# yuhogun0908/MISOnet

Hardware: AMD Instinct MI355X
Metric: utterances/sec MISO1->MVDR->MISO3, 6-mic 16kHz 4s (higher is better)
Workload: dtype f32w; 1 GPU; BASELINE configs[3]: synthetic 6-mic 16 kHz 4 s, full MISO1x6 -> align -> MVDRx2 -> MISO3x2; batch_per_gpu=16, global_batch=16, frames=1001, freq_bins=129, parallelism=utterance-shard x1

## Files before the change

### misonet_amd/csrc/kernels.hpp

```cpp
#pragma once
#include <hip/hip_runtime.h>
#include <stdint.h>
#include <stdlib.h>
#include "det_stats.hpp"

namespace mn {

constexpr int CK = 8;
constexpr int TT = 128;
constexpr int TW = 136;
constexpr int FT = 4;
constexpr float IN_EPS = 1e-5f;
constexpr float GLN_EPS = 1e-8f;

#ifdef MISONET_EXPERIMENTS
inline int exp_env(const char* name, int dflt) { const char* e = getenv(name); return e ? atoi(e) : dflt; }
#else
constexpr int exp_env(const char*, int dflt) { return dflt; }
#endif

inline int round_up(int x, int m) { return (x + m - 1) / m * m; }
inline int frames_pitch(int T) { return round_up(T, 32); }

struct ConvArgs {
// ... 41 lines not shown
    const unsigned id = blockIdx.x;
    const unsigned xcd = id & 7u, k = id >> 3;
    const unsigned per = (unsigned)(a.ntx * a.nty * a.ncg);
    const unsigned grp = k / per;
    unsigned tile = k - grp * per;
    r.n = (int)(grp * 8u + xcd);
    r.t_tile = (int)(tile % (unsigned)a.ntx);
    tile /= (unsigned)a.ntx;
    r.cg = (int)(tile % (unsigned)a.ncg);
    r.f_tile = (int)(tile / (unsigned)a.ncg);
    r.valid = r.n < a.nsamp;
  } else {
    r.t_tile = blockIdx.x; r.f_tile = blockIdx.y;
    r.n = blockIdx.z / a.ncg; r.cg = blockIdx.z - r.n * a.ncg;
    r.valid = true;
  }
  return r;
}
inline dim3 conv_grid(ConvArgs& a, int n_samples, int tt, int ft, int xcd) {
  a.ntx = (a.T + tt - 1) / tt; a.nty = (a.Fout + ft - 1) / ft; a.nsamp = n_samples; a.xcd = xcd;
  if (xcd) return dim3((unsigned)(8 * ((n_samples + 7) / 8) * a.ntx * a.nty * a.ncg), 1, 1);
  return dim3(a.ntx, a.nty, n_samples * a.ncg);
}
int conv_xcd_env();
int device_cus();
int conv_cop(int Cout);
int conv_rows(int sf, int tr2);
hipError_t launch_conv(const ConvArgs& a, int n_samples, hipStream_t s);
hipError_t launch_conv_w1d(const ConvArgs& a, int n_samples, hipStream_t s);
hipError_t conv_init();
hipError_t launch_conv_wino(const ConvArgs& a, int n_samples, hipStream_t s);
hipError_t conv_wino_init();
hipError_t launch_conv_few(const ConvArgs& a, int n_samples, hipStream_t s);
hipError_t conv_few_init();
hipError_t launch_conv_wino6(const ConvArgs& a, int n_samples, hipStream_t s);
hipError_t conv_wino6_init();
hipError_t launch_conv_bf16(const ConvArgs& a, int n_samples, hipStream_t s);
hipError_t conv_bf16_init();
hipError_t launch_conv_bf16_dma(const ConvArgs& a, int n_samples, hipStream_t s);
hipError_t launch_conv_wprep(const ConvArgs& a, const float* wf, int n_samples, hipStream_t s);
hipError_t conv_bf16_dma_init();
hipError_t launch_conv_bf16x6(const ConvArgs& a, int n_samples, hipStream_t s);
hipError_t launch_conv_wprep6(const ConvArgs& a, const float* wf6, int n_samples, hipStream_t s);
hipError_t conv_bf16x6_init();
long long conv_bf16x6_wps_bytes(int Cin, int Cout);
hipError_t launch_conv_x6_first(const ConvArgs& a, const void* wimg, int n_samples, hipStream_t s);

int tcn_part_slots(int T);
hipError_t launch_tcn_prepare(const float* raw, long long raw_bstride, int raw_c0, const dstat_t* raw_stats, int raw_sstride,
                              float* x, double2* x_part, int C, int T, int Tp, int n_samples, hipStream_t s,
                              int raw_oct3 = 0);
hipError_t launch_tcn_dw(const float* x, const double2* x_part, int x_np, const float* wdw , const float* prelu ,
                         float* d, double2* gln_part , int C, int T, int Tp, int dilation, int n_samples, hipStream_t s,
                         int norm_kind = 0, const float* nsc = nullptr, const float* nsh = nullptr, const float2* fstat = nullptr);
hipError_t launch_tcn_cln_stats(const float* x, float2* fstat, int C, int T, int Tp, int n_samples, hipStream_t s);
hipError_t launch_tcn_pw(const float* d, const double2* gln_part, const float* gamma, const float* beta,
                         const float* wpw , const float* residual ,
                         float* y, long long y_bstride, int y_c0, double2* y_part , int C, int T, int Tp,
                         int n_samples, hipStream_t s,
                         int y_oct3_cbuf = 0, int x6 = 0);

hipError_t launch_pack(const float2* src, int B, int Mseg, int T, int F, float* dst, long long dst_bstride, int Tp,
                       int c_re, int c_im, int nshift, hipStream_t s);
hipError_t launch_unpack(const float* src, long long src_bstride, int Tp, int S, int T, int F, float2* dst, int n_samples,
                         int* nan_flag, hipStream_t s);
hipError_t launch_export(const float* src, long long src_bstride, int c0, int C, int Fq, int T, int Tp,
                         const dstat_t* stats, int sstride, int ident_c, float* dst, int n_samples, hipStream_t s,
                         int oct = 0);
hipError_t launch_unpack_ex(const float* src, long long src_bstride, int Tp, int S, int T, int F, int c_re0, int c_im0, int mode,
                            int M, const int* sel, float2* dst, int n_out, int* nan_flag, hipStream_t s);
hipError_t launch_compose_sel(const int* shift_sel, const int* clean_sel, int B, int M, int S, int* out, hipStream_t s);
hipError_t launch_assemble3(const float* in1, long long in1_bstride, const float* out1, long long out1_bstride,
                            const int* sel, int B, int M, int S, int ref_ch, int F, int Tp, float* in3,
                            long long in3_bstride, hipStream_t s);

hipError_t launch_stft_pack(const float* wav, int B, int L, int Mw, int T, const float* twid, float* dst,
                            long long dst_bstride, int Tp, int F, int c_re, int c_im, int nshift, hipStream_t s);
hipError_t stft_init();
void stft_build_twiddles(float* tw);
int stft_twiddle_count();
hipError_t launch_istft(const void* spec, int N, int T, const float* itw, short* out_i16, float* out_f32, hipStream_t s);
hipError_t istft_init();
void istft_build_twiddles(float* tw);
int istft_twiddle_count();

struct CView {
  const float* re; const float* im;
  long long sb, sf, sm; int st;
};
enum { BF_MVDR = 0, BF_SOUDEN = 1, BF_GEV = 2 };
struct MvdrArgs {
  CView mix;
  const float* est;
  long long est_bstride;
  const int* sel;
  CView src;
  int S;
  int B, F, M, T, Tp;
  float epsi;
  int kind = BF_MVDR;
  int noise_mix = 0;
  int trace_norm = 0;
  int ban = 0;
  int bf_ref = 0;
  double condition = 0.0;
};
long long mvdr_ws_bytes(int B, int S, int F, int M);
// ... 132 lines not shown
```

### misonet_amd/csrc/net.hip

```cpp
#include "net.hpp"

#include <math.h>
#include <cmath>
#include <algorithm>
#include <stdarg.h>
#include <stdio.h>
#include <stdlib.h>
#include <string.h>

using namespace mn;

static thread_local char g_err[512] = "";
int mn::fail(int code, const char* fmt, ...) {
  va_list ap;
  va_start(ap, fmt);
  vsnprintf(g_err, sizeof(g_err), fmt, ap);
  va_end(ap);
  return code;
}

Prof mn::g_profs[MAX_DEV];
std::atomic<int> mn::g_prof_any{0};

static int find_tensor(const misonet_net* n, const std::string& name) {
// ... 153 lines not shown
    }
  n->taps.push_back({"enc0_conv", B_E0, 0, en[0], false});
  for (int b = 0; b < 7; ++b) {
    snprintf(nm, sizeof(nm), "enc%d", b);
    n->taps.push_back({nm, B_D0 + (6 - b), de[6 - b], en[b], true});
  }
  n->taps.push_back({"tcn_out", B_D0, 0, 128, false});
  for (int i = 0; i < 6; ++i) {
    snprintf(nm, sizeof(nm), "dec%d", i);
    n->taps.push_back({nm, B_D0 + i + 1, 0, de[i + 1], true});
  }
  n->taps.push_back({"dec6", B_OUT, 0, c.out_ch, false});
  static const int x6first_env = exp_env("MISONET_X6_FIRST", 1);
  for (std::vector<ConvL>* v : {&n->enc, &n->dec})
    for (ConvL& l : *v)
      for (int mode = 0; mode < CONV_NMODES; ++mode) {
        const ConvShape sh = {l.Cin, l.Cout, n->bufs[l.in_buf].F, n->bufs[l.out_buf].F, l.sf, l.padf, l.tr2, l.act, l.transposed,
                              l.ident_c, l.in_buf == B_IN, buf_oct(mode, l.in_buf), buf_oct(mode, l.out_buf)};
        l.kind[mode] = conv_mode_built(mode) ? conv_select(sh, mode) : ConvKind::DIRECT;
        if (l.kind[mode] == ConvKind::X6_FIRST && !x6first_env) l.kind[mode] = ConvKind::DIRECT;
      }
  return MISONET_OK;
}

static inline long long buf_floats(const misonet_net* n, int Tp, int b) {
  const long long e = (long long)n->bufs[b].C * n->bufs[b].F * Tp;
  return buf_oct(n, b) == 3 ? e + e / 2 : e;
}
long long mn::bstride(const misonet_net* n, const Layout& L, int b) {
  if (b == B_IN && L.in_ext_off >= 0) return L.in_ext_bstride;
  return b >= B_TXA ? buf_floats(n, L.Tp, b) : L.sample_stride;
}

static void buf_lifetime(int b, int& t0, int& t1) {
  if (b == B_IN) { t0 = 0; t1 = 16; }
  else if (b >= B_E0 && b <= B_E4) { t0 = t1 = 1 + (b - B_E0); }
  else if (b >= B_D0 && b <= B_D6) { const int i = b - B_D0; t0 = 7 - i; t1 = 9 + i; }
  else if (b >= B_X2 && b <= B_X6) { t0 = t1 = 9 + 2 + (b - B_X2); }
  else { t0 = 15; t1 = 16; }
}

Layout mn::make_layout(const misonet_net* n, int N, int T, bool ext_in) {
  Layout L;
  L.N = N; L.T = T; L.Tp = frames_pitch(T);
  long long so = 0;
  for (int b = 0; b < NBUF; ++b) {
    L.stats_off[b] = so;
    so += (long long)N * n->bufs[b].C * 2 * DS_NL;
  }
  const long long tslots = tcn_part_slots(T);
  so = (so + 1) & ~1LL;
  L.tcn_xs = so;  so += 15LL * N * 128 * tslots * 2;
  L.tcn_ps = so;  so += 14LL * N * 128 * tslots * 2;
  L.tcn_gln = so; so += 28LL * N * 32 * 2;
  L.stats_doubles = so;
  L.data_base = align_up(256 + so * 8, 256);
  {
    struct Rect { int b, t0, t1; long long off, size; };
    std::vector<Rect> placed;
    std::vector<int> order;
    for (int b = 0; b < B_TXA; ++b)
      if (!(ext_in && b == B_IN)) order.push_back(b);
    L.data_off[B_IN] = 0;
    std::sort(order.begin(), order.end(), [&](int x, int y) {
      const long long sx = buf_floats(n, L.Tp, x), sy = buf_floats(n, L.Tp, y);
      return sx != sy ? sx > sy : x < y;
    });
    long long top = 0;
    for (int b : order) {
      Rect r;
      r.b = b;
      r.size = align_up(buf_floats(n, L.Tp, b), 64);
      buf_lifetime(b, r.t0, r.t1);
      if (n->keep_taps) { r.t0 = 0; r.t1 = 16; }
      std::vector<long long> cand(1, 0);
      for (const Rect& q : placed)
        if (q.t0 <= r.t1 && r.t0 <= q.t1) cand.push_back(q.off + q.size);
      std::sort(cand.begin(), cand.end());
      for (long long o : cand) {
        bool ok = true;
        for (const Rect& q : placed)
          if (q.t0 <= r.t1 && r.t0 <= q.t1 && o < q.off + q.size && q.off < o + r.size) { ok = false; break; }
        if (ok) { r.off = o; break; }
      }
      placed.push_back(r);
      L.data_off[b] = r.off;
      top = std::max(top, r.off + r.size);
    }
    L.sample_stride = top;
  }
  long long d = (long long)N * L.sample_stride;
  for (int b = B_TXA; b < NBUF; ++b) {
    L.data_off[b] = d;
    d += align_up((long long)N * buf_floats(n, L.Tp, b), 64);
  }
  long long wmax = 0, cmax = 0;
  auto scan = [&](const std::vector<ConvL>& v) {
    for (const ConvL& c : v) {
      const long long g = (c.Cout + 31) / 32, k = (c.Cin + 15) / 16;
      wmax = std::max(wmax, g * k * (2LL * 9 * 2 * 32 * 16));
      wmax = std::max(wmax, conv_bf16x6_wps_bytes((c.Cin + 7) / 8 * 8, c.Cout));
      cmax = std::max(cmax, g * 32);
    }
  };
  scan(n->enc); scan(n->dec);
  L.wps_base = align_up(L.data_base + d * 4, 256);
  L.wps_nstride = wmax;
// ... 76 lines not shown
      if (e == hipSuccess) { ProfScope ps(s, PK_CONV); e = launch_conv_bf16_dma(a, nb, s); }
      break;
    case ConvKind::WINO6: { a.ww6 = c.img(n->w_dev, kind); ProfScope ps(s, PK_CONV); e = launch_conv_wino6(a, nb, s); } break;
#endif
    default: e = hipErrorInvalidValue; break;
  }
  if (e == hipErrorInvalidValue)
    return fail(MISONET_EINVAL, "conv kernel kind %d refuses the layer Cin=%d Cout=%d Fin=%d Fout=%d sf=%d padf=%d tr2=%d act=%d in_oct=%d out_oct=%d (mode %d)",
                (int)kind, a.Cin, a.Cout, a.Fin, a.Fout, a.sf, a.padf, a.tr2, a.act, a.in_oct, a.out_oct, n->precision);
  HIPCHK(e);
  return MISONET_OK;
}

static unsigned layout_stamp(const misonet_net* n, const Layout& L) {
  unsigned h = 2166136261u;
  auto mix = [&](unsigned long long v) { for (int i = 0; i < 8; ++i) { h ^= (unsigned)(v & 0xff); h *= 16777619u; v >>= 8; } };
  mix(n->keep_taps ? 1 : 0); mix((unsigned)n->precision); mix((unsigned)L.N); mix((unsigned)L.T); mix((unsigned long long)L.total_bytes);
  return h | 1u;
}

int mn::forward_planar(misonet_net* n, const Layout& L, void* ws, hipStream_t s) {
  HIPCHK(hipMemsetAsync(ws, 0, (size_t)(256 + L.tcn_xs * 8), s));
  HIPCHK(hipMemsetD32Async(reinterpret_cast<hipDeviceptr_t>(reinterpret_cast<char*>(ws) + 8), (int)layout_stamp(n, L), 1, s));
  static const int sub_env = exp_env("MISONET_SUBBATCH", 0);
  auto run_stack = [&](const std::vector<ConvL>& v) -> int {
    if (sub_env <= 0) {
      for (const ConvL& c : v) { int r = run_conv(n, L, ws, c, s); if (r) return r; }
      return MISONET_OK;
    }
    size_t i = 0;
    while (i < v.size()) {
      const int Fg = n->bufs[v[i].out_buf].F;
      size_t j = i;
      while (j < v.size() && n->bufs[v[j].out_buf].F == Fg) ++j;
      int sb = sub_env * (127 / (Fg > 0 ? Fg : 1));
      if (sb < 1) sb = 1;
      for (int n0 = 0; n0 < L.N; n0 += sb) {
        const int nb = (L.N - n0) < sb ? (L.N - n0) : sb;
        for (size_t k = i; k < j; ++k) { int r = run_conv(n, L, ws, v[k], s, n0, nb); if (r) return r; }
      }
      i = j;
    }
    return MISONET_OK;
  };
  { int r = run_stack(n->enc); if (r) return r; }
  {
    ProfScope ps_tcn(s, PK_TCN);
    const int N = L.N, T = L.T, Tp = L.Tp;
    double2* xs = reinterpret_cast<double2*>(stats_base(ws) + L.tcn_xs);
    double2* ps = reinterpret_cast<double2*>(stats_base(ws) + L.tcn_ps);
    double2* gl = reinterpret_cast<double2*>(stats_base(ws) + L.tcn_gln);
    const int tslots = tcn_part_slots(T);
    const long long per = (long long)N * 128 * tslots;
    const long long gper = (long long)N * 32;
    float* xa = buf_ptr(L, ws, B_TXA);
    float* xb = buf_ptr(L, ws, B_TXB);
    float* td = buf_ptr(L, ws, B_TD);
    float* tp = buf_ptr(L, ws, B_TP);
    const int skip_c0 = n->cfg.de_ch[0];
    HIPCHK(launch_tcn_prepare(buf_ptr(L, ws, B_D0), bstride(n, L, B_D0), skip_c0, stats_ptr(L, ws, B_D0),
                              n->bufs[B_D0].C, xa, xs, 128, T, Tp, N, s, buf_oct(n, B_D0) == 3));
    float* cur = xa;
    float* nxt = xb;
    static const int tcn_x6_env = exp_env("MISONET_TCN_X6", 1);
    const int tcn_x6 = (n->precision == 3 && tcn_x6_env) ? 1 : 0;
    for (int k = 0; k < 14; ++k) {
      const TcnBlock& tb = n->tcn[k];
      const float* W = n->w_dev;
      const int nk = n->cfg.tcn_norm;
      float2* fstat = reinterpret_cast<float2*>(reinterpret_cast<char*>(ws) + L.fstat_base);
      if (nk == 2) HIPCHK(launch_tcn_cln_stats(cur, fstat, 128, T, Tp, N, s));
      HIPCHK(launch_tcn_dw(cur, xs + k * per, k == 0 ? 1 : tslots, W + tb.h[0].o_dw, W + tb.h[0].o_prelu, td, gl + (2 * k) * gper,
                           128, T, Tp, tb.dilation, N, s, nk, W + tb.h[0].o_nsc, W + tb.h[0].o_nsh, fstat));
      HIPCHK(launch_tcn_pw(td, gl + (2 * k) * gper, W + tb.h[0].o_gamma, W + tb.h[0].o_beta, W + tb.h[0].o_pw,
                           nullptr, tp, 128LL * Tp, 0, ps + k * per, 128, T, Tp, N, s, 0, tcn_x6));
      if (nk == 2) HIPCHK(launch_tcn_cln_stats(tp, fstat, 128, T, Tp, N, s));
      HIPCHK(launch_tcn_dw(tp, ps + k * per, tslots, W + tb.h[1].o_dw, W + tb.h[1].o_prelu, td,
                           gl + (2 * k + 1) * gper, 128, T, Tp, tb.dilation, N, s, nk, W + tb.h[1].o_nsc, W + tb.h[1].o_nsh, fstat));
      const bool last = (k == 13);
      float* y = last ? buf_ptr(L, ws, B_D0) : nxt;
      HIPCHK(launch_tcn_pw(td, gl + (2 * k + 1) * gper, W + tb.h[1].o_gamma, W + tb.h[1].o_beta,
                           W + tb.h[1].o_pw, cur, y, last ? bstride(n, L, B_D0) : 128LL * Tp, 0,
                           xs + (k + 1) * per, 128, T, Tp, N, s, (last && buf_oct(n, B_D0) == 3) ? n->bufs[B_D0].C : 0, tcn_x6));
      float* t = cur; cur = nxt; nxt = t;
    }
  }
  { int r = run_stack(n->dec); if (r) return r; }
  return MISONET_OK;
}

extern "C" {

const char* misonet_strerror(int code) {
  switch (code) {
    case MISONET_OK: return "ok";
    case MISONET_EINVAL: return "invalid argument / unsupported geometry";
    case MISONET_ESTATE: return "invalid call order or missing tensor";
    case MISONET_EHIP: return "HIP runtime error";
    case MISONET_ENOMEM: return "workspace too small";
    case MISONET_ENAN: return "NaN in network output";
    default: return "unknown error";
  }
}
const char* misonet_last_error(void) { return g_err; }
int misonet_version(void) { return 560; }

int misonet_net_create(const misonet_cfg* cfg, misonet_net** out) {
  if (!cfg || !out) return fail(MISONET_EINVAL, "null argument");
  misonet_net* n = new misonet_net();
  n->cfg = *cfg;
  int r = build_plan(n);
  if (r) { delete n; return r; }
  *out = n;
  return MISONET_OK;
}

int misonet_net_destroy(misonet_net* n) {
  if (!n) return MISONET_OK;
  if (n->w_dev) (void)hipFree(n->w_dev);
  delete n;
  return MISONET_OK;
}

int misonet_net_num_tensors(const misonet_net* n) { return n ? (int)n->tensors.size() : 0; }
const char* misonet_net_tensor_name(const misonet_net* n, int i) {
  if (!n || i < 0 || i >= (int)n->tensors.size()) return nullptr;
  return n->tensors[i].name.c_str();
}
long long misonet_net_tensor_numel(const misonet_net* n, int i) {
  if (!n || i < 0 || i >= (int)n->tensors.size()) return -1;
  return n->tensors[i].numel;
}

int misonet_net_set_tensor(misonet_net* n, const char* key, const float* host, long long numel) {
// ... 343 lines not shown
```

### misonet_amd/csrc/net.hpp

```cpp
#pragma once
#include "conv_select.hpp"
#include "api_common.hpp"

#include <string>

namespace mn {

struct Tensor {
  std::string name;
  long long numel;
  std::vector<float> host;
  bool set = false;
};

enum { B_IN = 0, B_E0, B_E1, B_E2, B_E3, B_E4, B_D0, B_D1, B_D2, B_D3, B_D4, B_D5, B_D6, B_X2, B_X3, B_X4, B_X5, B_X6,
       B_OUT, B_TXA, B_TXB, B_TD, B_TP, NBUF };

struct BufSpec { int C = 0, F = 0; };

struct ConvL {
  int in_buf, in_c0, Cin, ident_c;
  int out_buf, out_c0, Cout;
  int sf, padf, tr2, act;
  bool transposed;
  int wt, bt;
  int cop, ncg;
  ConvKind kind[CONV_NMODES];
  long long img_off[CONV_NKIND];
  long long b_off = 0;
  float wscale = 1.f;
  const float* img(const float* w_dev, ConvKind k) const { return w_dev + img_off[(int)k]; }
};

struct TcnHalf {
  int dw, prelu, gamma, beta, pw; long long o_dw, o_prelu, o_gamma, o_beta, o_pw;
  int on[4] = {-1, -1, -1, -1};
  long long o_nsc = 0, o_nsh = 0;
};
struct TcnBlock { int dilation; TcnHalf h[2]; };

struct Tap { std::string name; int buf, c0, C; bool normalised; };

struct Layout {
  int N, T, Tp;
  long long data_off[NBUF];
  long long sample_stride;
  long long in_ext_off = -1;
  long long in_ext_bstride = 0;
  long long stats_off[NBUF];
  long long tcn_xs, tcn_ps, tcn_gln;
  long long stats_doubles;
  long long data_base;
  long long wps_base, wps_nstride;
  long long btab_base, btab_nstride;
  long long fstat_base;
  long long total_bytes;
};

}

struct misonet_net {
  misonet_cfg cfg;
  int S;
  mn::BufSpec bufs[mn::NBUF];
  std::vector<mn::Tensor> tensors;
  std::vector<mn::ConvL> enc, dec;
  std::vector<mn::TcnBlock> tcn;
  std::vector<mn::Tap> taps;
  float* w_dev = nullptr;
  bool committed = false;
  bool keep_taps = false;
  int precision = 3;
};

namespace mn {

inline long long align_up(long long x, long long a) { return (x + a - 1) / a * a; }

Layout make_layout(const misonet_net* n, int N, int T, bool ext_in = false);
long long bstride(const misonet_net* n, const Layout& L, int b);
inline float* buf_ptr(const Layout& L, void* ws, int b) {
  if (b == B_IN && L.in_ext_off >= 0) return reinterpret_cast<float*>(reinterpret_cast<char*>(ws) + L.in_ext_off);
  return reinterpret_cast<float*>(reinterpret_cast<char*>(ws) + L.data_base) + L.data_off[b];
}
int forward_planar(misonet_net* n, const Layout& L, void* ws, hipStream_t s);

}
```

### misonet_amd/csrc/tcn.hip

```cpp
#include "kernels.hpp"
#include "conv_epilogue.hpp"

namespace mn {

typedef float f32x16 __attribute__((ext_vector_type(16)));

__device__ inline double block_sum_256(double v, double* s_tmp ) {
#pragma unroll
  for (int m = 32; m >= 1; m >>= 1) v += __shfl_xor(v, m, 64);
  const int tid = threadIdx.x;
  __syncthreads();
  if ((tid & 63) == 0) s_tmp[tid >> 6] = v;
  __syncthreads();
  return s_tmp[0] + s_tmp[1] + s_tmp[2] + s_tmp[3];
}

__device__ inline double2 tpart_sum(const double2* p, int np) {
  double2 s = p[0];
#pragma unroll 8
  for (int i = 1; i < np; ++i) { const double2 q = p[i]; s.x += q.x; s.y += q.y; }
  return s;
}

__device__ inline void in_params(double2 st, int T, float& mean, float& rstd) {
  const double m = st.x / (double)T;
  double var = st.y / (double)T - m * m;
  var = var > 0.0 ? var : 0.0;
  mean = (float)m;
  rstd = (float)(1.0 / sqrt(var + (double)IN_EPS));
}

__global__ __launch_bounds__(256) void tcn_prepare_k(const float* raw, long long raw_bstride, int raw_c0,
                                                     const dstat_t* raw_stats, int raw_sstride, float* x,
                                                     double2* x_part, int nps, int C, int T, int Tp, int raw_oct3) {
  __shared__ double s_tmp[4];
  const int c = blockIdx.x, n = blockIdx.y;
  float mean, rstd;
  {
    const dstat_t* st = raw_stats + ((long long)n * raw_sstride + raw_c0 + c) * (2 * DS_NL);
    in_params(make_double2(dstat_read(st), dstat_read(st + DS_NL)), T, mean, rstd);
  }
  const float* src = raw + (long long)n * raw_bstride + (long long)(raw_c0 + c) * Tp;
  const unsigned short* so = reinterpret_cast<const unsigned short*>(raw + (long long)n * raw_bstride);
  const int ch = raw_c0 + c;
  const long long part_e = (long long)(raw_sstride >> 3) * Tp * 8;
  float* dst = x + ((long long)n * C + c) * Tp;
  double s1 = 0.0, s2 = 0.0;
  for (int t = threadIdx.x; t < T; t += 256) {
    float r;
    if (raw_oct3) {
      const long long e = ((long long)(ch >> 3) * Tp + t) * 8 + (ch & 7);
      r = (__uint_as_float((unsigned)so[e] << 16) + __uint_as_float((unsigned)so[part_e + e] << 16)) +
          __uint_as_float((unsigned)so[2 * part_e + e] << 16);
    } else {
      r = src[t];
    }
    const float v = (r - mean) * rstd;
    dst[t] = v;
    s1 += v;
    s2 += (double)v * v;
  }
  s1 = block_sum_256(s1, s_tmp);
  s2 = block_sum_256(s2, s_tmp);
  if (threadIdx.x == 0) x_part[((long long)n * C + c) * nps] = make_double2(s1, s2);
}

constexpr int DW_MAXT = 2048;
constexpr int DW_HALO = 64;
constexpr int DW_SEG = DW_MAXT - 2 * DW_HALO;
template <int NORM>
__global__ __launch_bounds__(256) void tcn_dw_k(const float* x, const double2* x_part, int x_np, int nps,
                                                const float* wdw, const float* prelu, float* d, double2* gln_part,
                                                int C, int T, int Tp, int dil, int seg_f, const float* nsc, const float* nsh,
                                                const float2* fstat) {
  __shared__ double s_tmp[4][2];
  extern __shared__ __align__(16) float s_a_dyn[];
  const int row_f = seg_f + 2 * DW_HALO;
  const int lane = threadIdx.x & 63, wave = threadIdx.x >> 6;
  const int c = blockIdx.x * 4 + wave, n = blockIdx.y;
  float sc, sh, mu = 0.f;
  if (NORM == 0) {
    float mean, rstd;
    in_params(tpart_sum(x_part + ((long long)n * C + c) * nps, x_np), T, mean, rstd);
    sc = rstd; sh = 0.f; mu = mean;
  } else if (NORM == 1) {
    __shared__ double s_g[4];
    double a1 = 0.0, a2 = 0.0;
    for (int r = threadIdx.x; r < C; r += 256) {
      const double2 q = tpart_sum(x_part + ((long long)n * C + r) * nps, x_np);
      a1 += q.x; a2 += q.y;
    }
    a1 = block_sum_256(a1, s_g);
    a2 = block_sum_256(a2, s_g);
    const double cnt = (double)C * (double)T;
    const double gm = a1 / cnt;
    double gv = a2 / cnt - gm * gm;
    gv = gv > 0.0 ? gv : 0.0;
    const float rstd = (float)(1.0 / sqrt(gv + (double)GLN_EPS));
    sc = nsc[c] * rstd;
    sh = nsh[c];
    mu = (float)gm;
  } else if (NORM == 3) {
    sc = nsc[c]; sh = nsh[c];
  } else {
    sc = nsc[c]; sh = nsh[c];
  }
  const float2* fs = NORM == 2 ? fstat + (long long)n * Tp : nullptr;
  const float w0 = wdw[c * 3 + 0], w1 = wdw[c * 3 + 1], w2 = wdw[c * 3 + 2];
  const float slope = prelu[0];
  const float* src = x + ((long long)n * C + c) * Tp;
  float* dst = d + ((long long)n * C + c) * Tp;
  float* a = s_a_dyn + wave * row_f;
  const int Tq = (T + 3) & ~3;
  double r1 = 0.0, r2 = 0.0;
  for (int ts = 0; ts < Tq; ts += seg_f) {
    if (ts) __syncthreads();
    for (int j = lane * 4; j < row_f; j += 256) {
      const int t = ts - DW_HALO + j;
      float4 o = make_float4(0.f, 0.f, 0.f, 0.f);
      if (t >= 0 && t < Tq) {
        float4 v = *reinterpret_cast<const float4*>(src + t);
        if (NORM == 2) {
          const float4 f01 = *reinterpret_cast<const float4*>(fs + t), f23 = *reinterpret_cast<const float4*>(fs + t + 2);
          v.x = (v.x - f01.x) * f01.y; v.y = (v.y - f01.z) * f01.w;
          v.z = (v.z - f23.x) * f23.y; v.w = (v.w - f23.z) * f23.w;
        }
        o.x = (t + 0 < T) ? elu_fast(fmaf(v.x - mu, sc, sh)) : 0.f;
        o.y = (t + 1 < T) ? elu_fast(fmaf(v.y - mu, sc, sh)) : 0.f;
        o.z = (t + 2 < T) ? elu_fast(fmaf(v.z - mu, sc, sh)) : 0.f;
        o.w = (t + 3 < T) ? elu_fast(fmaf(v.w - mu, sc, sh)) : 0.f;
      }
      *reinterpret_cast<float4*>(a + j) = o;
    }
    __syncthreads();
    const int te = (ts + seg_f < Tq) ? ts + seg_f : Tq;
    float s1 = 0.f, s2 = 0.f;
    for (int t = ts + lane * 4; t < te; t += 256) {
      float o[4];
#pragma unroll
      for (int i = 0; i < 4; ++i) {
        const int tc = t + i;
        const int j = tc - ts + DW_HALO;
        float acc = w1 * a[j];
        acc = fmaf(w0, a[j - dil], acc);
        acc = fmaf(w2, a[j + dil], acc);
        acc = acc > 0.f ? acc : slope * acc;
        o[i] = acc;
        if (tc < T) { s1 += acc; s2 = fmaf(acc, acc, s2); }
      }
      *reinterpret_cast<float4*>(dst + t) = make_float4(o[0], o[1], o[2], o[3]);
    }
    r1 += (double)s1;
    r2 += (double)s2;
  }
// ... 193 lines not shown
  __amdgpu_buffer_rsrc_t rs_o[3];
  {
    const unsigned long long po = reinterpret_cast<unsigned long long>(y) + (unsigned long long)n * y_bstride * 4ull +
                                  (unsigned long long)(y_c0 >> 3) * OP16;
    const unsigned long long pb = (unsigned long long)(y_cbuf >> 3) * OP16;
    const unsigned nrec = Y_OCT3 ? (unsigned)(C >> 3) * OP16 : 0u;
    rs_o[0] = make_rsrc_e(po, nrec);
    rs_o[1] = make_rsrc_e(po + pb, nrec);
    rs_o[2] = make_rsrc_e(po + 2 * pb, nrec);
  }
  float s1[16], s2[16], piv[16];
#pragma unroll
  for (int r = 0; r < 16; ++r) {
    s1[r] = 0.f; s2[r] = 0.f;
    piv[r] = __shfl(acc[0][r] + rv[0][r], lane & 32, 64);
  }
#pragma unroll
  for (int s = 0; s < 4; ++s) {
    const int t = t0 + s * 32 + l31;
    const bool ok = t < T;
    const float m = ok ? 1.f : 0.f;
    const unsigned vo = ok ? (unsigned)((wave * 32 + 4 * half) * Tp + t) * 4u : 0x80000000u;
    float vrow[16];
#pragma unroll
    for (int r = 0; r < 16; ++r) {
      const int co_off = (r & 3) + 8 * (r >> 2);
      const float v = acc[s][r] + rv[s][r];
      vrow[r] = v;
      if (!Y_OCT3)
        __builtin_amdgcn_raw_buffer_store_b32(__builtin_bit_cast(unsigned, v), rs_y, vo + (unsigned)(co_off * Tp) * 4u, 0, 0);
      const float vm = (v - piv[r]) * m;
      s1[r] += vm;
      s2[r] = fmaf(vm, vm, s2[r]);
    }
    if (Y_OCT3)
      store_oct_row<3>(vrow, rs_o, (unsigned)t * 16u + (unsigned)(4 * wave + half) * OP16, OP16, ok, ok);
  }
  if (y_part) {
    const float x1 = reduce16_halfwave(s1, lane);
    const float x2 = reduce16_halfwave(s2, lane);
    if ((lane & 16) == 0) {
      const int q = lane & 15;
      const int co = wave * 32 + (q & 3) + 8 * (q >> 2) + 4 * half;
      float pq = piv[0];
#pragma unroll
      for (int r = 1; r < 16; ++r) pq = (q == r) ? piv[r] : pq;
      const double c = (double)pq, S1 = (double)x1, S2 = (double)x2;
      const double nv = (double)((T - t0) < PW_TT ? (T - t0) : PW_TT);
      y_part[((long long)n * C + co) * nps + blockIdx.x] = make_double2(S1 + nv * c, S2 + 2.0 * c * S1 + nv * c * c);
    }
  }
}

int tcn_part_slots(int T) { return (T + PW_TT - 1) / PW_TT; }

hipError_t launch_tcn_prepare(const float* raw, long long raw_bstride, int raw_c0, const dstat_t* raw_stats,
                              int raw_sstride, float* x, double2* x_part, int C, int T, int Tp, int n_samples,
                              hipStream_t s, int raw_oct3) {
  hipLaunchKernelGGL(tcn_prepare_k, dim3(C, n_samples), dim3(256), 0, s, raw, raw_bstride, raw_c0, raw_stats,
                     raw_sstride, x, x_part, tcn_part_slots(T), C, T, Tp, raw_oct3);
  return hipGetLastError();
}

__global__ __launch_bounds__(256) void tcn_cln_stats_k(const float* x, float2* fstat, int C, int T, int Tp) {
  const int t = blockIdx.x * 256 + threadIdx.x, n = blockIdx.y;
  if (t >= Tp) return;
  float2 o = make_float2(0.f, 0.f);
  if (t < T) {
    const float* p = x + (long long)n * C * Tp + t;
    float m = 0.f;
    for (int c = 0; c < C; ++c) m += p[(long long)c * Tp];
    m /= (float)C;
    float v = 0.f;
    for (int c = 0; c < C; ++c) { const float dd = p[(long long)c * Tp] - m; v = fmaf(dd, dd, v); }
    v /= (float)C;
    o = make_float2(m, 1.f / sqrtf(v + GLN_EPS));
  }
  fstat[(long long)n * Tp + t] = o;
}

hipError_t launch_tcn_cln_stats(const float* x, float2* fstat, int C, int T, int Tp, int n_samples, hipStream_t s) {
  hipLaunchKernelGGL(tcn_cln_stats_k, dim3((Tp + 255) / 256, n_samples), dim3(256), 0, s, x, fstat, C, T, Tp);
  return hipGetLastError();
}

hipError_t launch_tcn_dw(const float* x, const double2* x_part, int x_np, const float* wdw, const float* prelu, float* d,
                         double2* gln_part, int C, int T, int Tp, int dilation, int n_samples, hipStream_t s, int norm_kind,
                         const float* nsc, const float* nsh, const float2* fstat) {
  if (dilation < 1 || dilation > DW_HALO) return hipErrorInvalidValue;
  if (C % 4) return hipErrorInvalidValue;
  if (norm_kind < 0 || norm_kind > 3 || (norm_kind && (!nsc || !nsh)) || (norm_kind == 2 && !fstat)) return hipErrorInvalidValue;
  const int tq = (T + 3) & ~3;
  const int seg_f = tq < DW_SEG ? tq : DW_SEG;
  const dim3 g(C / 4, n_samples);
  const size_t lds = (size_t)4 * (seg_f + 2 * DW_HALO) * sizeof(float);
#define MN_DW(K) hipLaunchKernelGGL(tcn_dw_k<K>, g, dim3(256), lds, s, x, x_part, x_np, tcn_part_slots(T), wdw, prelu, d, gln_part, \
                                    C, T, Tp, dilation, seg_f, nsc, nsh, fstat)
  if (norm_kind == 0) MN_DW(0); else if (norm_kind == 1) MN_DW(1); else if (norm_kind == 2) MN_DW(2); else MN_DW(3);
#undef MN_DW
  return hipGetLastError();
}

hipError_t launch_tcn_pw(const float* d, const double2* gln_part, const float* gamma, const float* beta,
                         const float* wpw, const float* residual, float* y, long long y_bstride, int y_c0,
                         double2* y_part, int C, int T, int Tp, int n_samples, hipStream_t s, int y_oct3_cbuf, int x6) {
  if (C != 128) return hipErrorInvalidValue;
  const dim3 g((T + PW_TT - 1) / PW_TT, n_samples);
  const int nps = tcn_part_slots(T);
  if (y_oct3_cbuf) {
    if ((y_c0 & 7) || (y_oct3_cbuf & 7)) return hipErrorInvalidValue;
    if (x6) hipLaunchKernelGGL((tcn_pw_k<true, true>), g, dim3(256), 0, s, d, gln_part, gamma, beta, wpw, residual, y,
                               y_bstride, y_c0, y_part, nps, T, Tp, y_oct3_cbuf);
    else hipLaunchKernelGGL((tcn_pw_k<true, false>), g, dim3(256), 0, s, d, gln_part, gamma, beta, wpw, residual, y,
                            y_bstride, y_c0, y_part, nps, T, Tp, y_oct3_cbuf);
  } else {
    if (x6) hipLaunchKernelGGL((tcn_pw_k<false, true>), g, dim3(256), 0, s, d, gln_part, gamma, beta, wpw, residual, y,
                               y_bstride, y_c0, y_part, nps, T, Tp, 0);
    else hipLaunchKernelGGL((tcn_pw_k<false, false>), g, dim3(256), 0, s, d, gln_part, gamma, beta, wpw, residual, y,
                            y_bstride, y_c0, y_part, nps, T, Tp, 0);
  }
  return hipGetLastError();
}

}
```

Before: 149.1 utt/s.

## Fuse first TCN depthwise conv with pointwise conv, defer gLN into next norm

Adds a fused kernel that computes the first half-block's depthwise conv, PReLU and gamma scaling in LDS and feeds it straight into the pointwise MFMA GEMM. This removes the intermediate depthwise activation round-trip through global memory and one launch per TCN block. The global-LayerNorm statistics are folded algebraically into the following depthwise kernel's instance-norm scale (new NORM==4 path), using pivot-shifted partial sums for numerical stability. Beta is dropped, which is valid only because the next instance norm cancels per-channel offsets. The cost is a larger, more register- and LDS-hungry kernel and a more fragile chain of statistics.

```diff
diff --git a/misonet_amd/csrc/kernels.hpp b/misonet_amd/csrc/kernels.hpp
--- a/misonet_amd/csrc/kernels.hpp
+++ b/misonet_amd/csrc/kernels.hpp
@@ -117,7 +117,12 @@
                               int raw_oct3 = 0);
 hipError_t launch_tcn_dw(const float* x, const double2* x_part, int x_np, const float* wdw , const float* prelu ,
                          float* d, double2* gln_part , int C, int T, int Tp, int dilation, int n_samples, hipStream_t s,
-                         int norm_kind = 0, const float* nsc = nullptr, const float* nsh = nullptr, const float2* fstat = nullptr);
+                         int norm_kind = 0, const float* nsc = nullptr, const float* nsh = nullptr, const float2* fstat = nullptr,
+                         const double2* p_gln = nullptr);
+hipError_t launch_tcn_ds(const float* x, const double2* x_part, int x_np, const float* wdw , const float* prelu ,
+                         const float* gamma, const float* wpw, float* p, double2* p_part ,
+                         double2* gln_part , int C, int T, int Tp, int dilation, int n_samples, hipStream_t s,
+                         int x6 = 0, const double2* pivot_gln = nullptr);
 hipError_t launch_tcn_cln_stats(const float* x, float2* fstat, int C, int T, int Tp, int n_samples, hipStream_t s);
 hipError_t launch_tcn_pw(const float* d, const double2* gln_part, const float* gamma, const float* beta,
                          const float* wpw , const float* residual ,
diff --git a/misonet_amd/csrc/net.hip b/misonet_amd/csrc/net.hip
--- a/misonet_amd/csrc/net.hip
+++ b/misonet_amd/csrc/net.hip
@@ -229,7 +229,8 @@
   so = (so + 1) & ~1LL;
   L.tcn_xs = so;  so += 15LL * N * 128 * tslots * 2;
   L.tcn_ps = so;  so += 14LL * N * 128 * tslots * 2;
-  L.tcn_gln = so; so += 28LL * N * 32 * 2;
+  L.tcn_g0 = (int)std::max(32LL, tslots);
+  L.tcn_gln = so; so += 14LL * N * (L.tcn_g0 + 32) * 2;
   L.stats_doubles = so;
   L.data_base = align_up(256 + so * 8, 256);
   {
@@ -412,7 +413,8 @@
     double2* gl = reinterpret_cast<double2*>(stats_base(ws) + L.tcn_gln);
     const int tslots = tcn_part_slots(T);
     const long long per = (long long)N * 128 * tslots;
-    const long long gper = (long long)N * 32;
+    const long long g0per = (long long)N * L.tcn_g0;
+    const long long gper = g0per + (long long)N * 32;
     float* xa = buf_ptr(L, ws, B_TXA);
     float* xb = buf_ptr(L, ws, B_TXB);
     float* td = buf_ptr(L, ws, B_TD);
@@ -424,22 +426,33 @@
     float* nxt = xb;
     static const int tcn_x6_env = exp_env("MISONET_TCN_X6", 1);
     const int tcn_x6 = (n->precision == 3 && tcn_x6_env) ? 1 : 0;
+    static const int tcn_fuse = exp_env("MISONET_TCN_FUSE", 1);
     for (int k = 0; k < 14; ++k) {
       const TcnBlock& tb = n->tcn[k];
       const float* W = n->w_dev;
       const int nk = n->cfg.tcn_norm;
       float2* fstat = reinterpret_cast<float2*>(reinterpret_cast<char*>(ws) + L.fstat_base);
       if (nk == 2) HIPCHK(launch_tcn_cln_stats(cur, fstat, 128, T, Tp, N, s));
-      HIPCHK(launch_tcn_dw(cur, xs + k * per, k == 0 ? 1 : tslots, W + tb.h[0].o_dw, W + tb.h[0].o_prelu, td, gl + (2 * k) * gper,
-                           128, T, Tp, tb.dilation, N, s, nk, W + tb.h[0].o_nsc, W + tb.h[0].o_nsh, fstat));
-      HIPCHK(launch_tcn_pw(td, gl + (2 * k) * gper, W + tb.h[0].o_gamma, W + tb.h[0].o_beta, W + tb.h[0].o_pw,
-                           nullptr, tp, 128LL * Tp, 0, ps + k * per, 128, T, Tp, N, s, 0, tcn_x6));
-      if (nk == 2) HIPCHK(launch_tcn_cln_stats(tp, fstat, 128, T, Tp, N, s));
-      HIPCHK(launch_tcn_dw(tp, ps + k * per, tslots, W + tb.h[1].o_dw, W + tb.h[1].o_prelu, td,
-                           gl + (2 * k + 1) * gper, 128, T, Tp, tb.dilation, N, s, nk, W + tb.h[1].o_nsc, W + tb.h[1].o_nsh, fstat));
+      double2* g0 = gl + k * gper;
+      double2* g1 = g0 + g0per;
+      if (nk == 0 && tcn_fuse) {
+        HIPCHK(launch_tcn_ds(cur, xs + k * per, k == 0 ? 1 : tslots, W + tb.h[0].o_dw, W + tb.h[0].o_prelu, W + tb.h[0].o_gamma,
+                             W + tb.h[0].o_pw, tp, ps + k * per, g0, 128, T, Tp, tb.dilation, N, s, tcn_x6,
+                             k ? g0 - gper : nullptr));
+        HIPCHK(launch_tcn_dw(tp, ps + k * per, tslots, W + tb.h[1].o_dw, W + tb.h[1].o_prelu, td, g1, 128, T, Tp, tb.dilation,
+                             N, s, 4, nullptr, nullptr, nullptr, g0));
+      } else {
+        HIPCHK(launch_tcn_dw(cur, xs + k * per, k == 0 ? 1 : tslots, W + tb.h[0].o_dw, W + tb.h[0].o_prelu, td, g0,
+                             128, T, Tp, tb.dilation, N, s, nk, W + tb.h[0].o_nsc, W + tb.h[0].o_nsh, fstat));
+        HIPCHK(launch_tcn_pw(td, g0, W + tb.h[0].o_gamma, W + tb.h[0].o_beta, W + tb.h[0].o_pw,
+                             nullptr, tp, 128LL * Tp, 0, ps + k * per, 128, T, Tp, N, s, 0, tcn_x6));
+        if (nk == 2) HIPCHK(launch_tcn_cln_stats(tp, fstat, 128, T, Tp, N, s));
+        HIPCHK(launch_tcn_dw(tp, ps + k * per, tslots, W + tb.h[1].o_dw, W + tb.h[1].o_prelu, td,
+                             g1, 128, T, Tp, tb.dilation, N, s, nk, W + tb.h[1].o_nsc, W + tb.h[1].o_nsh, fstat));
+      }
       const bool last = (k == 13);
       float* y = last ? buf_ptr(L, ws, B_D0) : nxt;
-      HIPCHK(launch_tcn_pw(td, gl + (2 * k + 1) * gper, W + tb.h[1].o_gamma, W + tb.h[1].o_beta,
+      HIPCHK(launch_tcn_pw(td, g1, W + tb.h[1].o_gamma, W + tb.h[1].o_beta,
                            W + tb.h[1].o_pw, cur, y, last ? bstride(n, L, B_D0) : 128LL * Tp, 0,
                            xs + (k + 1) * per, 128, T, Tp, N, s, (last && buf_oct(n, B_D0) == 3) ? n->bufs[B_D0].C : 0, tcn_x6));
       float* t = cur; cur = nxt; nxt = t;
diff --git a/misonet_amd/csrc/net.hpp b/misonet_amd/csrc/net.hpp
--- a/misonet_amd/csrc/net.hpp
+++ b/misonet_amd/csrc/net.hpp
@@ -49,6 +49,7 @@
   long long in_ext_bstride = 0;
   long long stats_off[NBUF];
   long long tcn_xs, tcn_ps, tcn_gln;
+  int tcn_g0;
   long long stats_doubles;
   long long data_base;
   long long wps_base, wps_nstride;
diff --git a/misonet_amd/csrc/tcn.hip b/misonet_amd/csrc/tcn.hip
--- a/misonet_amd/csrc/tcn.hip
+++ b/misonet_amd/csrc/tcn.hip
@@ -72,7 +72,7 @@
 __global__ __launch_bounds__(256) void tcn_dw_k(const float* x, const double2* x_part, int x_np, int nps,
                                                 const float* wdw, const float* prelu, float* d, double2* gln_part,
                                                 int C, int T, int Tp, int dil, int seg_f, const float* nsc, const float* nsh,
-                                                const float2* fstat) {
+                                                const float2* fstat, const double2* p_gln) {
   __shared__ double s_tmp[4][2];
   extern __shared__ __align__(16) float s_a_dyn[];
   const int row_f = seg_f + 2 * DW_HALO;
@@ -100,6 +100,20 @@
     sc = nsc[c] * rstd;
     sh = nsh[c];
     mu = (float)gm;
+  } else if (NORM == 4) {
+    const double2 st = tpart_sum(x_part + ((long long)n * C + c) * nps, x_np);
+    const double2 gs = tpart_sum(p_gln + (long long)n * nps, nps);
+    const double cnt = (double)C * (double)T;
+    const double gm = gs.x / cnt;
+    double gv = gs.y / cnt - gm * gm;
+    gv = gv < 0.0 ? 0.0 : gv;
+    const double r = 1.0 / sqrt(gv + (double)GLN_EPS);
+    const double m = st.x / (double)T;
+    double var = st.y / (double)T - m * m;
+    var = var < 0.0 ? 0.0 : var;
+    mu = (float)m;
+    sc = (float)(r / sqrt(r * r * var + (double)IN_EPS));
+    sh = 0.f;
   } else if (NORM == 3) {
     sc = nsc[c]; sh = nsh[c];
   } else {
@@ -399,7 +413,304 @@
   }
 }
 
+constexpr int DS_AW = PW_TT + 2 * DW_HALO;
+
+__device__ __forceinline__ float4 ds_row4(const float* p, bool al4) {
+  if (al4) return *reinterpret_cast<const float4*>(p);
+  return make_float4(p[0], p[1], p[2], p[3]);
+}
+
+__device__ __forceinline__ float ds_tap(float slope, float ac, float al, float ar, float4 cw) {
+  float acc = cw.y * ac;
+  acc = fmaf(cw.x, al, acc);
+  acc = fmaf(cw.z, ar, acc);
+  return acc > 0.f ? acc : slope * acc;
+}
+
+__device__ __forceinline__ float ds_keep(float v, unsigned mask) {
+  return __builtin_bit_cast(float, __builtin_bit_cast(unsigned, v) & mask);
+}
+
+template <bool X6>
+__global__ __launch_bounds__(256) void tcn_ds_k(const float* x, const double2* x_part, int x_np, int nps, const float* wdw,
+                                                const float* prelu, const float* gamma, const float* wt ,
+                                                float* y, double2* y_part, double2* gln_part, int T, int Tp, int dil,
+                                                const double2* piv_part) {
+  constexpr int C = 128;
+  __shared__ __align__(16) float s_a[PW_KC][DS_AW];
+  __shared__ __align__(16) float4 s_cw[C];
+  __shared__ float2 s_in[C];
+  __shared__ double s_red[4][2];
+  const int tid = threadIdx.x, lane = tid & 63, wave = tid >> 6;
+  const int half = lane >> 5, l31 = lane & 31;
+  const int t0 = blockIdx.x * PW_TT, n = blockIdx.y;
+  const float* xn = x + (long long)n * C * Tp;
+  if (tid < C) {
+    float mean, rstd;
+    in_params(tpart_sum(x_part + ((long long)n * C + tid) * nps, x_np), T, mean, rstd);
+    s_in[tid] = make_float2(mean, rstd);
+    s_cw[tid] = make_float4(wdw[tid * 3 + 0], wdw[tid * 3 + 1], wdw[tid * 3 + 2], gamma[tid]);
+  }
+  const float slope = prelu[0];
+  const bool al4 = (dil & 3) == 0;
+  const float cpv = piv_part ? (float)(tpart_sum(piv_part + (long long)n * nps, nps).x / ((double)C * (double)T)) : 0.f;
+  const int ec = tid >> 4, eq = tid & 15;
+  const int qlo = (DW_HALO - dil) >> 2, qhi = (DW_HALO + PW_TT + dil + 3) >> 2;
+  const int ni = (qhi - qlo + 15) >> 4;
+  const int tq0 = t0 - DW_HALO + 4 * (qlo + eq), tq1 = tq0 + 64, tq2 = tq0 + 128, tq3 = tq0 + 192;
+  const float* xe = xn + ec * Tp;
+  const float* xp0 = xe + ((unsigned)tq0 < (unsigned)Tp ? tq0 : 0);
+  const float* xp1 = xe + ((unsigned)tq1 < (unsigned)Tp ? tq1 : 0);
+  const float* xp2 = xe + ((unsigned)tq2 < (unsigned)Tp ? tq2 : 0);
+  const float* xp3 = xe + ((unsigned)tq3 < (unsigned)Tp ? tq3 : 0);
+  float* ae = &s_a[ec][4 * (qlo + eq)];
+  float4 xr0, xr1, xr2, xr3 = make_float4(0.f, 0.f, 0.f, 0.f);
+#define DS_XISSUE(K0)                                                                                            \
+  {                                                                                                              \
+    const int ko_ = (K0) * Tp;                                                                                   \
+    xr0 = *reinterpret_cast<const float4*>(xp0 + ko_);                                                           \
+    xr1 = *reinterpret_cast<const float4*>(xp1 + ko_);                                                           \
+    xr2 = *reinterpret_cast<const float4*>(xp2 + ko_);                                                           \
+    if (ni > 3) xr3 = *reinterpret_cast<const float4*>(xp3 + ko_);                                               \
+  }
+#define DS_AELU(XV, TQ, I)                                                                                       \
+  {                                                                                                              \
+    float4 o_;                                                                                                   \
+    o_.x = elu_fast((unsigned)((TQ) + 0) < (unsigned)T ? (XV.x - ms_.x) * ms_.y : 0.f);                          \
+    o_.y = elu_fast((unsigned)((TQ) + 1) < (unsigned)T ? (XV.y - ms_.x) * ms_.y : 0.f);                          \
+    o_.z = elu_fast((unsigned)((TQ) + 2) < (unsigned)T ? (XV.z - ms_.x) * ms_.y : 0.f);                          \
+    o_.w = elu_fast((unsigned)((TQ) + 3) < (unsigned)T ? (XV.w - ms_.x) * ms_.y : 0.f);                          \
+    *reinterpret_cast<float4*>(ae + 64 * (I)) = o_;                                                              \
+  }
+#define DS_ACOMMIT(K0)                                                                                           \
+  {                                                                                                              \
+    const float2 ms_ = s_in[(K0) + ec];                                                                          \
+    DS_AELU(xr0, tq0, 0) DS_AELU(xr1, tq1, 1) DS_AELU(xr2, tq2, 2)                                               \
+    if (ni > 3) DS_AELU(xr3, tq3, 3)                                                                             \
+  }
+  f32x16 acc[4];
+#pragma unroll
+  for (int s = 0; s < 4; ++s)
+#pragma unroll
+    for (int r = 0; r < 16; ++r) acc[s][r] = 0.f;
+  double r1 = 0.0, r2 = 0.0;
+  __syncthreads();
+
+  if constexpr (X6) {
+    typedef __bf16 bf16x8_t __attribute__((ext_vector_type(8)));
+    __shared__ __align__(16) u32x4_t s_x[2][3][2][PW_TT];
+    const int so = tid >> 7, sf = tid & 127;
+    const bool tok = t0 + sf < T;
+    const float* wl = wt + (long long)(8 * half) * C + wave * 32 + l31;
+    float win[2][8];
+    u32x4_t A[3];
+#define X6_WISSUE(SL, K0)                                                                                        \
+  _Pragma("unroll") for (int c = 0; c < 8; ++c) win[SL][c] = wl[((K0) + c) * C];
+#define X6_DCOMMIT(BUF, SL, K0)                                                                                  \
+  {                                                                                                              \
+    float g_[8], s1_ = 0.f, s2_ = 0.f;                                                                           \
+    _Pragma("unroll") for (int c = 0; c < 8; ++c) {                                                              \
+      const float4 cw_ = s_cw[(K0) + 8 * so + c];                                                                \
+      const float* ar_ = &s_a[8 * so + c][DW_HALO + sf];                                                         \
+      float d_ = ds_tap(slope, ar_[0], ar_[-dil], ar_[dil], cw_);                                                       \
+      d_ = tok ? d_ : 0.f;                                                                                       \
+      s1_ += d_; s2_ = fmaf(d_, d_, s2_);                                                                        \
+      g_[c] = tok ? (d_ - cpv) * cw_.w : 0.f;                                                                    \
+    }                                                                                                            \
+    r1 += (double)s1_; r2 += (double)s2_;                                                                        \
+    u32x4_t h_, m_, l_;                                                                                          \
+    _Pragma("unroll") for (int i = 0; i < 4; ++i) {                                                              \
+      unsigned hh_, mm_, ll_;                                                                                    \
+      split3_pair_t(g_[2 * i], g_[2 * i + 1], hh_, mm_, ll_);                                                    \
+      h_[i] = hh_; m_[i] = mm_; l_[i] = ll_;                                                                     \
+    }                                                                                                            \
+    s_x[BUF][0][so][sf] = h_; s_x[BUF][1][so][sf] = m_; s_x[BUF][2][so][sf] = l_;                                \
+    _Pragma("unroll") for (int i = 0; i < 4; ++i) {                                                              \
+      unsigned hh_, mm_, ll_;                                                                                    \
+      split3_pair_t(win[SL][2 * i], win[SL][2 * i + 1], hh_, mm_, ll_);                                          \
+      A[0][i] = hh_; A[1][i] = mm_; A[2][i] = ll_;                                                               \
+    }                                                                                                            \
+  }
+    X6_WISSUE(0, 0)
+    X6_WISSUE(1, 16)
+    DS_XISSUE(0)
+    DS_ACOMMIT(0)
+    __syncthreads();
+    X6_DCOMMIT(0, 0, 0)
+    __syncthreads();
+#define X6_STEP(KC, SL)                                                                                          \
+    {                                                                                                            \
+      if ((KC) + 2 < C / 16) X6_WISSUE(SL, ((KC) + 2) * 16)      \
+      if ((KC) + 1 < C / 16) DS_XISSUE(((KC) + 1) * 16)                                                          \
+      const bf16x8_t Ah = __builtin_bit_cast(bf16x8_t, A[0]), Am = __builtin_bit_cast(bf16x8_t, A[1]),           \
+                     Al = __builtin_bit_cast(bf16x8_t, A[2]);                                                    \
+      _Pragma("unroll") for (int s = 0; s < 4; ++s) {                                                            \
+        const bf16x8_t Bh = __builtin_bit_cast(bf16x8_t, s_x[SL][0][half][s * 32 + l31]);                        \
+        const bf16x8_t Bm = __builtin_bit_cast(bf16x8_t, s_x[SL][1][half][s * 32 + l31]);                        \
+        const bf16x8_t Bl = __builtin_bit_cast(bf16x8_t, s_x[SL][2][half][s * 32 + l31]);                        \
+                                                                  \
+        acc[s] = __builtin_amdgcn_mfma_f32_32x32x16_bf16(Al, Bh, acc[s], 0, 0, 0);                               \
+        acc[s] = __builtin_amdgcn_mfma_f32_32x32x16_bf16(Ah, Bl, acc[s], 0, 0, 0);                               \
+        acc[s] = __builtin_amdgcn_mfma_f32_32x32x16_bf16(Am, Bm, acc[s], 0, 0, 0);                               \
+        acc[s] = __builtin_amdgcn_mfma_f32_32x32x16_bf16(Am, Bh, acc[s], 0, 0, 0);                               \
+        acc[s] = __builtin_amdgcn_mfma_f32_32x32x16_bf16(Ah, Bm, acc[s], 0, 0, 0);                               \
+        acc[s] = __builtin_amdgcn_mfma_f32_32x32x16_bf16(Ah, Bh, acc[s], 0, 0, 0);                               \
+      }                                                                                                          \
+      if ((KC) + 1 < C / 16) {                                                                                   \
+        DS_ACOMMIT(((KC) + 1) * 16)           \
+        __syncthreads();                                                                                         \
+        X6_DCOMMIT((SL) ^ 1, (SL) ^ 1, ((KC) + 1) * 16)                                                          \
+        __syncthreads();                                                                                         \
+      }                                                                                                          \
+    }
+#pragma unroll
+    for (int kp = 0; kp < C / 32; ++kp) {
+      X6_STEP(2 * kp, 0)
+      X6_STEP(2 * kp + 1, 1)
+    }
+#undef X6_STEP
+#undef X6_WISSUE
+#undef X6_DCOMMIT
+  } else {
+    __shared__ __align__(16) float s_g[2][PW_KC][PW_TT];
+    __shared__ __align__(16) float s_w[2][PW_KC][C];
+    const int sq = tid & 31, sg = tid >> 5;
+    const int tg = t0 + 4 * sq;
+    const unsigned mk0 = tg + 0 < T ? ~0u : 0u, mk1 = tg + 1 < T ? ~0u : 0u, mk2 = tg + 2 < T ? ~0u : 0u, mk3 = tg + 3 < T ? ~0u : 0u;
+    float4 wi0, wi1;
+#define DS_WISSUE(K0)                                                                                            \
+  wi0 = *reinterpret_cast<const float4*>(wt + (long long)((K0) + sg) * C + 4 * sq);                              \
+  wi1 = *reinterpret_cast<const float4*>(wt + (long long)((K0) + sg + 8) * C + 4 * sq);
+#define DS_DROW(BUF, K0, I, WV)                                                                                  \
+  {                                                                                                              \
+    const float4 cw_ = s_cw[(K0) + sg + 8 * (I)];                                                                \
+    const float* ar_ = &s_a[sg + 8 * (I)][DW_HALO + 4 * sq];                                                     \
+    const float4 c4_ = *reinterpret_cast<const float4*>(ar_);                                                    \
+    const float4 l4_ = ds_row4(ar_ - dil, al4), r4_ = ds_row4(ar_ + dil, al4);                                   \
+    float4 d_;                                                                                                   \
+    d_.x = ds_keep(ds_tap(slope, c4_.x, l4_.x, r4_.x, cw_), mk0);                                         \
+    d_.y = ds_keep(ds_tap(slope, c4_.y, l4_.y, r4_.y, cw_), mk1);                                         \
+    d_.z = ds_keep(ds_tap(slope, c4_.z, l4_.z, r4_.z, cw_), mk2);                                         \
+    d_.w = ds_keep(ds_tap(slope, c4_.w, l4_.w, r4_.w, cw_), mk3);                                         \
+    s1_ += (d_.x + d_.y) + (d_.z + d_.w);                                                                        \
+    s2_ = fmaf(d_.x, d_.x, s2_); s2_ = fmaf(d_.y, d_.y, s2_);                                                    \
+    s2_ = fmaf(d_.z, d_.z, s2_); s2_ = fmaf(d_.w, d_.w, s2_);                                                    \
+    *reinterpret_cast<float4*>(&s_g[BUF][sg + 8 * (I)][4 * sq]) =                                                \
+        make_float4(ds_keep((d_.x - cpv) * cw_.w, mk0), ds_keep((d_.y - cpv) * cw_.w, mk1),                      \
+                    ds_keep((d_.z - cpv) * cw_.w, mk2), ds_keep((d_.w - cpv) * cw_.w, mk3));                     \
+    *reinterpret_cast<float4*>(&s_w[BUF][sg + 8 * (I)][4 * sq]) = WV;                                            \
+  }
+#define DS_DCOMMIT(BUF, K0)                                                                                      \
+  {                                                                                                              \
+    float s1_ = 0.f, s2_ = 0.f;                                                                                  \
+    DS_DROW(BUF, K0, 0, wi0) DS_DROW(BUF, K0, 1, wi1)                                                            \
+    r1 += (double)s1_; r2 += (double)s2_;                                                                        \
+  }
+    DS_WISSUE(0)
+    DS_XISSUE(0)
+    DS_ACOMMIT(0)
+    __syncthreads();
+    DS_DCOMMIT(0, 0)
+    __syncthreads();
+#pragma unroll
+    for (int kc = 0; kc < C / PW_KC; ++kc) {
+      const int buf = kc & 1;
+      if (kc + 1 < C / PW_KC) {
+        DS_WISSUE((kc + 1) * PW_KC)
+        DS_XISSUE((kc + 1) * PW_KC)
+      }
+#pragma unroll
+      for (int kk = 0; kk < PW_KC; kk += 2) {
+        const float av = s_w[buf][kk + half][wave * 32 + l31];
+#pragma unroll
+        for (int s = 0; s < 4; ++s) {
+          const float bv = s_g[buf][kk + half][s * 32 + l31];
+          acc[s] = __builtin_amdgcn_mfma_f32_32x32x2f32(av, bv, acc[s], 0, 0, 0);
+        }
+      }
+      if (kc + 1 < C / PW_KC) {
+        DS_ACOMMIT((kc + 1) * PW_KC)
+        __syncthreads();
+        DS_DCOMMIT(buf ^ 1, (kc + 1) * PW_KC)
+        __syncthreads();
+      }
+    }
+#undef DS_WISSUE
+#undef DS_DROW
+#undef DS_DCOMMIT
+  }
+#undef DS_XISSUE
+#undef DS_AELU
+#undef DS_ACOMMIT
+
+#pragma unroll
+  for (int m = 32; m >= 1; m >>= 1) {
+    r1 += __shfl_xor(r1, m, 64);
+    r2 += __shfl_xor(r2, m, 64);
+  }
+  if (lane == 0) { s_red[wave][0] = r1; s_red[wave][1] = r2; }
+  __syncthreads();
+  if (tid == 0)
+    gln_part[(long long)n * gridDim.x + blockIdx.x] = make_double2((s_red[0][0] + s_red[1][0]) + (s_red[2][0] + s_red[3][0]),
+                                                                   (s_red[0][1] + s_red[1][1]) + (s_red[2][1] + s_red[3][1]));
+
+  float* yn = y + (long long)n * C * Tp;
+  const unsigned long long pa = reinterpret_cast<unsigned long long>(yn);
+  const unsigned plo = __builtin_amdgcn_readfirstlane((unsigned)pa);
+  const unsigned phi = __builtin_amdgcn_readfirstlane((unsigned)(pa >> 32));
+  const __amdgpu_buffer_rsrc_t rs_y = __builtin_amdgcn_make_buffer_rsrc(
+      reinterpret_cast<void*>(((unsigned long long)phi << 32) | plo), 0,
+      __builtin_amdgcn_readfirstlane((int)((unsigned)C * (unsigned)Tp * 4u)), 0x00020000);
+  float s1[16], s2[16], piv[16];
+#pragma unroll
+  for (int r = 0; r < 16; ++r) {
+    s1[r] = 0.f; s2[r] = 0.f;
+    piv[r] = __shfl(acc[0][r], lane & 32, 64);
+  }
+#pragma unroll
+  for (int s = 0; s < 4; ++s) {
+    const int t = t0 + s * 32 + l31;
+    const bool ok = t < T;
+    const float m = ok ? 1.f : 0.f;
+    const unsigned vo = ok ? (unsigned)((wave * 32 + 4 * half) * Tp + t) * 4u : 0x80000000u;
+#pragma unroll
+    for (int r = 0; r < 16; ++r) {
+      const int co_off = (r & 3) + 8 * (r >> 2);
+      const float v = acc[s][r];
+      __builtin_amdgcn_raw_buffer_store_b32(__builtin_bit_cast(unsigned, v), rs_y, vo + (unsigned)(co_off * Tp) * 4u, 0, 0);
+      const float vm = (v - piv[r]) * m;
+      s1[r] += vm;
+      s2[r] = fmaf(vm, vm, s2[r]);
+    }
+  }
+  const float x1 = reduce16_halfwave(s1, lane);
+  const float x2 = reduce16_halfwave(s2, lane);
+  if ((lane & 16) == 0) {
+    const int q = lane & 15;
+    const int co = wave * 32 + (q & 3) + 8 * (q >> 2) + 4 * half;
+    float pq = piv[0];
+#pragma unroll
+    for (int r = 1; r < 16; ++r) pq = (q == r) ? piv[r] : pq;
+    const double c = (double)pq, S1 = (double)x1, S2 = (double)x2;
+    const double nv = (double)((T - t0) < PW_TT ? (T - t0) : PW_TT);
+    y_part[((long long)n * C + co) * nps + blockIdx.x] = make_double2(S1 + nv * c, S2 + 2.0 * c * S1 + nv * c * c);
+  }
+}
+
 int tcn_part_slots(int T) { return (T + PW_TT - 1) / PW_TT; }
+
+hipError_t launch_tcn_ds(const float* x, const double2* x_part, int x_np, const float* wdw, const float* prelu,
+                         const float* gamma, const float* wpw, float* p, double2* p_part, double2* gln_part, int C, int T,
+                         int Tp, int dilation, int n_samples, hipStream_t s, int x6, const double2* pivot_gln) {
+  if (C != 128) return hipErrorInvalidValue;
+  if (dilation < 1 || dilation > DW_HALO) return hipErrorInvalidValue;
+  const dim3 g(tcn_part_slots(T), n_samples);
+  if (x6) hipLaunchKernelGGL(tcn_ds_k<true>, g, dim3(256), 0, s, x, x_part, x_np, tcn_part_slots(T), wdw, prelu, gamma, wpw, p,
+                             p_part, gln_part, T, Tp, dilation, pivot_gln);
+  else hipLaunchKernelGGL(tcn_ds_k<false>, g, dim3(256), 0, s, x, x_part, x_np, tcn_part_slots(T), wdw, prelu, gamma, wpw, p,
+                          p_part, gln_part, T, Tp, dilation, pivot_gln);
+  return hipGetLastError();
+}
 
 hipError_t launch_tcn_prepare(const float* raw, long long raw_bstride, int raw_c0, const dstat_t* raw_stats,
                               int raw_sstride, float* x, double2* x_part, int C, int T, int Tp, int n_samples,
@@ -433,17 +744,19 @@
 
 hipError_t launch_tcn_dw(const float* x, const double2* x_part, int x_np, const float* wdw, const float* prelu, float* d,
                          double2* gln_part, int C, int T, int Tp, int dilation, int n_samples, hipStream_t s, int norm_kind,
-                         const float* nsc, const float* nsh, const float2* fstat) {
+                         const float* nsc, const float* nsh, const float2* fstat, const double2* p_gln) {
   if (dilation < 1 || dilation > DW_HALO) return hipErrorInvalidValue;
   if (C % 4) return hipErrorInvalidValue;
-  if (norm_kind < 0 || norm_kind > 3 || (norm_kind && (!nsc || !nsh)) || (norm_kind == 2 && !fstat)) return hipErrorInvalidValue;
+  if (norm_kind < 0 || norm_kind > 4) return hipErrorInvalidValue;
+  if (norm_kind == 4 ? !p_gln : ((norm_kind && (!nsc || !nsh)) || (norm_kind == 2 && !fstat))) return hipErrorInvalidValue;
   const int tq = (T + 3) & ~3;
   const int seg_f = tq < DW_SEG ? tq : DW_SEG;
   const dim3 g(C / 4, n_samples);
   const size_t lds = (size_t)4 * (seg_f + 2 * DW_HALO) * sizeof(float);
 #define MN_DW(K) hipLaunchKernelGGL(tcn_dw_k<K>, g, dim3(256), lds, s, x, x_part, x_np, tcn_part_slots(T), wdw, prelu, d, gln_part, \
-                                    C, T, Tp, dilation, seg_f, nsc, nsh, fstat)
-  if (norm_kind == 0) MN_DW(0); else if (norm_kind == 1) MN_DW(1); else if (norm_kind == 2) MN_DW(2); else MN_DW(3);
+                                    C, T, Tp, dilation, seg_f, nsc, nsh, fstat, p_gln)
+  if (norm_kind == 0) MN_DW(0); else if (norm_kind == 1) MN_DW(1); else if (norm_kind == 2) MN_DW(2);
+  else if (norm_kind == 3) MN_DW(3); else MN_DW(4);
 #undef MN_DW
   return hipGetLastError();
 }
```

Result: no change. 149.7 utt/s, median of 6 (+0.4%).
